# this-Demir/3D-Ray-Tracer-Vulkan

Hardware: AMD Instinct MI355X
Metric: Mrays/s at 1920×1080×4-bounce, 50k-tri scene; 1/2/4/8 GPU + %HBM roofline (higher is better)
Workload: dtype f32

## Files before the change

3d-ray-tracer-vulkan_amd/csrc/rt_trace.hip:

```cpp
#include <algorithm>
#include <cstdio>
#include <cstdlib>
#include <cstring>

#include "rt_internal.h"

namespace rtamd {

namespace {

constexpr float kTMin = 0.001f;
constexpr float kTMax = 10000.0f;
constexpr int   kMaxRejectTriples = 1 << 16;

struct V3 { float x, y, z; };

__device__ __forceinline__ V3 vadd(V3 a, V3 b) { return {a.x + b.x, a.y + b.y, a.z + b.z}; }
__device__ __forceinline__ V3 vsub(V3 a, V3 b) { return {a.x - b.x, a.y - b.y, a.z - b.z}; }
__device__ __forceinline__ V3 vmul(V3 a, V3 b) { return {a.x * b.x, a.y * b.y, a.z * b.z}; }
__device__ __forceinline__ V3 vscale(V3 a, float s) { return {a.x * s, a.y * s, a.z * s}; }
__device__ __forceinline__ float vdot(V3 a, V3 b) { return (a.x * b.x + a.y * b.y) + a.z * b.z; }
__device__ __forceinline__ V3 vcross(V3 a, V3 b) {
    return {a.y * b.z - a.z * b.y, a.z * b.x - a.x * b.z, a.x * b.y - a.y * b.x};
}
__device__ __forceinline__ V3 vnormalize(V3 a) {
    const float l = sqrtf(vdot(a, a));
    return {a.x / l, a.y / l, a.z / l};
}

__device__ __forceinline__ uint32_t pcg(uint32_t v) {
    const uint32_t s = v * 747796405u + 2891336453u;
    const uint32_t w = ((s >> ((s >> 28u) + 4u)) ^ s) * 277803737u;
    return (w >> 22u) ^ w;
}
__device__ __forceinline__ float rnd(uint32_t& seed) {
    seed = pcg(seed);
    return (float)seed / 4294967296.0f;
}

__device__ __forceinline__ V3 rnd_in_sphere(uint32_t& seed) {
    seed = pcg(pcg(pcg(seed)));
    for (int it = 0; it < kMaxRejectTriples; ++it) {
        const float a = rnd(seed);
        const float b = rnd(seed);
        const float c = rnd(seed);
        const V3 p = {a * 2.0f - 1.0f, b * 2.0f - 1.0f, c * 2.0f - 1.0f};
        if (vdot(p, p) < 1.0f) return p;
    }
    return {0.0f, 0.0f, 0.0f};
}

__device__ __forceinline__ uint8_t unorm8(float c) {
    return c > 0.0f ? (c < 1.0f ? (uint8_t)__builtin_rintf(c * 255.0f) : (uint8_t)255) : (uint8_t)0;
}

__device__ __forceinline__ int frame_row(const TraceArgs& a, int f, int ly) {
    if (a.band_list) return a.y0 + a.band_list[f * a.list_stride + ly / a.band_h] * a.band_h + ly % a.band_h;
    return a.y0 + ((ly / a.band_h) * a.band_stride + a.band_off) * a.band_h + ly % a.band_h;
}

__device__ __forceinline__ void primary_ray_seeded(const TraceArgs& a, int f, int x, int y, uint32_t& seed, V3& o,
                                                   V3& d);
__device__ __forceinline__ void primary_ray(const TraceArgs& a, int f, int x, int y, uint32_t& seed, V3& o, V3& d) {
    seed = (uint32_t)(y * a.width + x);
    primary_ray_seeded(a, f, x, y, seed, o, d);
}

__device__ __forceinline__ void primary_ray_seeded(const TraceArgs& a, int f, int x, int y, uint32_t& seed, V3& o,
                                                   V3& d) {
    const float u = ((float)x + rnd(seed)) / (float)a.width;
    const float v = ((float)(a.height - 1 - y) + rnd(seed)) / (float)a.height;
    const CamF& c = a.cams[f];
    const V3 cam_o = {c.ox, c.oy, c.oz};
    const V3 cam_l = {c.lx, c.ly, c.lz};
    const V3 cam_h = {c.hx, c.hy, c.hz};
    const V3 cam_v = {c.vx, c.vy, c.vz};
    o = cam_o;
    d = vnormalize(vsub(vadd(vadd(cam_l, vscale(cam_h, u)), vscale(cam_v, v)), cam_o));
}

typedef float f2 __attribute__((ext_vector_type(2)));

__device__ __forceinline__ void slab(float4 A, float4 B, V3 o, V3 inv, float& te, bool& ind) {
    const f2 oxy = {o.x, o.y}, ixy = {inv.x, inv.y};
    const f2 t0 = (f2{A.x, A.y} - oxy) * ixy;
    const f2 t1 = (f2{B.x, B.y} - oxy) * ixy;
    const float t0x = t0.x, t1x = t1.x, t0y = t0.y, t1y = t1.y;
    const float t0z = (A.z - o.z) * inv.z, t1z = (B.z - o.z) * inv.z;
    te = fmaxf(fmaxf(fminf(t0x, t1x), fminf(t0y, t1y)), fminf(t0z, t1z));
    const float tx = fminf(fminf(fmaxf(t0x, t1x), fmaxf(t0y, t1y)), fmaxf(t0z, t1z));
    ind = tx > te && tx > kTMin;
}

__device__ __forceinline__ bool tri_test(float4 P0, float4 P1, float4 P2, V3 o, V3 d, float& t) {
    const V3 v0 = {P0.x, P0.y, P0.z};
    const V3 e1 = {P1.x, P1.y, P1.z};
    const V3 e2 = {P2.x, P2.y, P2.z};
    const V3 pv = vcross(d, e2);
    const float det = vdot(e1, pv);
    if (det > -0.00001f && det < 0.00001f) return false;
    const float inv_det = 1.0f / det;
    const V3 s = vsub(o, v0);
    const float uu = inv_det * vdot(s, pv);
    if (uu < 0.0f || uu > 1.0f) return false;
    const V3 q = vcross(s, e1);
    const float vv = inv_det * vdot(d, q);
    if (vv < 0.0f || (uu + vv) > 1.0f) return false;
    t = inv_det * vdot(e2, q);
    return t > kTMin;
}

__device__ __forceinline__ void pin(float4& q) { asm volatile("" : "+v"(q.x), "+v"(q.y), "+v"(q.z), "+v"(q.w)); }

template <bool COUNT>
__device__ __forceinline__ int node_step(const float4* __restrict__ nodes, const float4* __restrict__ leafs,
                                         int i, bool& leaf, V3 o, V3 d, V3 inv, float& closest, int& hit,
                                         unsigned long long& c_node, unsigned long long& c_tri) {
    const float4 A = nodes[2 * i];
    const float4 B = nodes[2 * i + 1];
    float4 P0, P1, P2;
    if (leaf) {
        P0 = leafs[3 * i + 0];
        P1 = leafs[3 * i + 1];
        P2 = leafs[3 * i + 2];
        pin(P0);
        pin(P1);
        pin(P2);
    }
    float te;
    bool ind;
    slab(A, B, o, inv, te, ind);
    const bool hb = ind && te < closest;
    if (COUNT && hb && !leaf) c_node += 2;
    if (hb && leaf) {
        if (COUNT) ++c_tri;
        float t;
        if (tri_test(P0, P1, P2, o, d, t) && t < closest) {
            closest = t;
            hit = __float_as_int(P0.w);
        }
    }
    const uint32_t aw = __float_as_uint(A.w), bw = __float_as_uint(B.w);
    leaf = hb ? (bw & 1u) : (aw >> 31);
    return hb ? i + 1 : (int)(aw & 0x7FFFFFFFu);
}

__device__ __forceinline__ V3 hit_normal(const float4* __restrict__ norms, int hit, V3 d) {
    const float4 N = norms[kShadeStride * hit];
    V3 n = {N.x, N.y, N.z};
    if (vdot(d, n) > 0.0f) n = {-n.x, -n.y, -n.z};
    return n;
}

__device__ __forceinline__ void sphere_tests(const float4* __restrict__ sph, int n, V3 o, V3 d,
                                             float& closest, int& hit) {
    const float qa = vdot(d, d);
    for (int k = 0; k < n; ++k) {
        const float4 S = sph[2 * k];
        const V3 oc = {o.x - S.x, o.y - S.y, o.z - S.z};
        const float hb = vdot(oc, d);
        const float qc = vdot(oc, oc) - S.w * S.w;
        const float disc = hb * hb - qa * qc;
        if (!(disc >= 0.0f)) continue;
        const float sq = sqrtf(disc);
        float root = (-hb - sq) / qa;
        if (!(root > kTMin && root < closest)) {
            root = (-hb + sq) / qa;
            if (!(root > kTMin && root < closest)) continue;
        }
        closest = root;
        hit = -2 - k;
    }
}

__device__ __forceinline__ V3 sphere_normal(float4 S, V3 hp, V3 d) {
    V3 n = {(hp.x - S.x) / S.w, (hp.y - S.y) / S.w, (hp.z - S.z) / S.w};
    if (vdot(d, n) > 0.0f) n = {-n.x, -n.y, -n.z};
    return n;
}

__device__ __forceinline__ bool scatter(float4 M, V3 d, V3 n, uint32_t& seed, V3& nd) {
    if (M.w == 0.0f) {
        const V3 ru = vnormalize(rnd_in_sphere(seed));
        V3 sd = vadd(n, ru);
        if (sqrtf(vdot(sd, sd)) < 0.0001f) sd = n;
        nd = vnormalize(sd);
        return true;
    }
    if (M.w == 1.0f || M.w == 2.0f) {
        const float fuzz = (M.w == 2.0f) ? 0.3f : 0.0f;
        const V3 di = vnormalize(d);
        const float k = 2.0f * vdot(n, di);
        const V3 refl = vsub(di, vscale(n, k));
        const V3 p = rnd_in_sphere(seed);
        nd = vnormalize(vadd(refl, vscale(p, fuzz)));
        return vdot(nd, n) > 0.0f;
    }
    nd = d;
    return false;
}

__device__ __forceinline__ V3 sky_color(V3 d) {
    const V3 ud = vnormalize(d);
    const float t = 0.5f * (ud.y + 1.0f);
    const float omt = 1.0f - t;
    return {omt * 1.0f + t * 0.5f, omt * 1.0f + t * 0.7f, omt * 1.0f + t * 1.0f};
}

__device__ __forceinline__ void write_pixel(const TraceArgs& a, int lx, int ly, V3 fin) {
    const V3 g = {sqrtf(fin.x), sqrtf(fin.y), sqrtf(fin.z)};
    const size_t p = (size_t)ly * (size_t)a.tw + (size_t)lx;
    if (a.out_rgba) a.out_rgba[p] = make_uchar4(unorm8(g.x), unorm8(g.y), unorm8(g.z), 255);
    if (a.out_rad) {
        a.out_rad[3 * p + 0] = g.x;
        a.out_rad[3 * p + 1] = g.y;
        a.out_rad[3 * p + 2] = g.z;
    }
}

constexpr int kFeatExtBit = 16;

template <int FEAT>
__device__ __forceinline__ void finish_pixel(const TraceArgs& a, int lx, int ly, V3 fin) {
    if ((FEAT & kFeatExtBit) && a.out_lin) {
        float* lin = a.out_lin + 3 * ((size_t)ly * (size_t)a.tw + (size_t)lx);
        lin[0] = fin.x;
        lin[1] = fin.y;
        lin[2] = fin.z;
        return;
    }
    if ((FEAT & kFeatExtBit) && (a.ext & kExtAccumulate)) {
        float* acc = a.accum + 3 * ((size_t)ly * (size_t)a.tw + (size_t)lx);
        const float nf = (float)(a.frame_count + 1);
        const V3 sum = a.frame_count == 0 ? fin : V3{acc[0] + fin.x, acc[1] + fin.y, acc[2] + fin.z};
        acc[0] = sum.x;
        acc[1] = sum.y;
        acc[2] = sum.z;
        fin = {sum.x / nf, sum.y / nf, sum.z / nf};
    }
    write_pixel(a, lx, ly, fin);
}

__device__ __forceinline__ void flush_counters(Counters* c, unsigned long long s, unsigned long long n,
                                               unsigned long long t, unsigned long long m) {
// ... 346 lines not shown
        const uint64_t CI = __ballot(cand && !lf);
        if (room < 2 && ((CI >> k) & 1ull)) {
            pos = lane_i(node, k);
            pos_leaf = false;
            return false;
        }
        const bool sel = cand && (lf || lane == k || 2 * (lanes_below(CI) + 1) <= room - kFReserve);
        bool hL = false, hR = false;
        uint4 cL = e, cR = e;
        if (sel) {
            if (lf) {
                const float4 P0 = leafs[3 * node + 0];
                const float4 P1 = leafs[3 * node + 1];
                const float4 P2 = leafs[3 * node + 2];
                float t;
                const bool v = tri_test(P0, P1, P2, o, d, t);
                e.y = __float_as_uint(P0.w);
                e.w = v ? __float_as_uint(t) : 0x7F800000u;
            } else {
                const float4 Q0 = pairs[4 * node + 0];
                const float4 Q1 = pairs[4 * node + 1];
                const float4 Q2 = pairs[4 * node + 2];
                const float4 Q3 = pairs[4 * node + 3];
                float teL, teR;
                bool indL, indR;
                slab(Q0, Q1, o, inv, teL, indL);
                slab(make_float4(Q0.w, Q1.w, Q2.w, 0.f), Q2, o, inv, teR, indR);
                const uint32_t rw = __float_as_uint(Q3.x);
                hL = indL && teL < closest;
                hR = indR && teR < closest;
                cL = make_uint4((uint32_t)(node + 1) | (__float_as_uint(Q3.y) != 0u ? 0x80000000u : 0u), rw & kIdx,
                                __float_as_uint(teL), kUnres);
                cR = make_uint4(rw, e.y, __float_as_uint(teR), kUnres);
                e.w = 0u;
            }
        }
        const bool reg = in && lane >= k;
        const uint64_t RM = __ballot(reg), LM = __ballot(hL), RRM = __ballot(hR);
        const int P = lanes_below(RM) + lanes_below(LM) + lanes_below(RRM);
        const int ntop = top - (nl - k) + __popcll(RM) + __popcll(LM) + __popcll(RRM);
        if (reg) {
            F[ntop - 1 - P] = e;
            if (hL) F[ntop - 2 - P] = cL;
            if (hR) F[ntop - 2 - (hL ? 1 : 0) - P] = cR;
        }
        top = ntop;
    }
    pos = end;
    return true;
}


__device__ __forceinline__ void diag_stamp(unsigned long long* rec, int which) {
    unsigned long long t;
    asm volatile("s_memrealtime %0\n\ts_waitcnt lgkmcnt(0)" : "=s"(t) :: "memory");
    if ((threadIdx.x & 63) == 0) {
        rec[which] = t;
        if (which == 0) {
            unsigned hw, xcc;
            asm volatile("s_getreg_b32 %0, hwreg(HW_REG_HW_ID)" : "=s"(hw));
            asm volatile("s_getreg_b32 %0, hwreg(HW_REG_XCC_ID)" : "=s"(xcc));
            rec[2] = ((unsigned long long)xcc << 32) | hw;
            rec[3] = ((unsigned long long)(blockIdx.y * gridDim.x + blockIdx.x) << 8) | (threadIdx.x >> 6);
        }
    }
}

constexpr int kDiagWords = 8;
constexpr int kFeatCoopTail = 8;
constexpr int kFeatExt = kFeatExtBit;
constexpr int kFeatFrontier = 32;

constexpr int kFeatFused = 64;
constexpr int kFeatWin32 = 128;
constexpr int kFeatPad = 256;
constexpr int kFeatQ1 = 4096;
constexpr int kFeatQ2 = 8192;
constexpr int kFeatHalf = 2048;
constexpr int kFeatWide = 1024;
constexpr int kFeatAccel = 512;
constexpr int kFeatQuery = 16384;
constexpr int kFeatSolo = 32768;
constexpr unsigned kHeavyLaneMark = kLearnHeavyMark;

__device__ __forceinline__ void store_hit(float4* h, float t, int tri, V3 n, V3 p) {
    h[0] = make_float4(t, __int_as_float(tri), n.x, n.y);
    h[1] = make_float4(n.z, p.x, p.y, p.z);
}
__device__ __forceinline__ bool finite3(V3 a) {
    return fabsf(a.x) < __builtin_inff() && fabsf(a.y) < __builtin_inff() && fabsf(a.z) < __builtin_inff();
}

template <bool COUNT>
__device__ __forceinline__ void heavy_pixel(const TraceArgs& a, int f, int lx, int ly, int lyo, uint4* F) {
    const int lane = threadIdx.x & 63;
    const int end = a.scene.end;
    unsigned long long c_seg = 0, c_node = 0, c_tri = 0, c_mat = 0;
    if (lx < a.tw && ly < a.th && (a.list_stride == 0 || a.band_list[f * a.list_stride + ly / a.band_h] >= 0)) {
        uint32_t seed;
        V3 o, d;
        primary_ray(a, f, a.x0 + lx, frame_row(a, f, ly), seed, o, d);
        V3 att = {1.0f, 1.0f, 1.0f};
        V3 fin = {0.0f, 0.0f, 0.0f};
        int rounds = 0;
        for (int b = 0; b < a.max_bounces; ++b) {
            float closest = kTMax;
            int hit = -1;
            const V3 inv = {1.0f / d.x, 1.0f / d.y, 1.0f / d.z};
            if (COUNT) {
                ++c_seg;
                if (end > 0) ++c_node;
            }
            if (end > 0) {
                int p = 0;
                bool pl = false;
                if (!frontier_walk<COUNT>(a.scene.nodes, a.scene.leafs, a.scene.pairs, end, p, pl, o, d, inv, closest,
                                          hit, c_node, c_tri, F, rounds))
                    while (p < end) p = node_step<COUNT>(a.scene.nodes, a.scene.leafs, p, pl, o, d, inv, closest, hit,
                                                         c_node, c_tri);
            }
            if (hit < 0) {
                fin = vmul(att, sky_color(d));
                break;
            }
            if (COUNT) ++c_mat;
            const V3 hp = vadd(o, vscale(d, closest));
            const V3 nrm = hit_normal(a.scene.norms, hit, d);
            const float4 M = a.scene.mats[kShadeStride * hit];
            V3 nd;
            if (!scatter(M, d, nrm, seed, nd)) break;
            att = vmul(att, V3{M.x, M.y, M.z});
            o = hp;
            d = nd;
        }
        if (lane == 0) write_pixel(a, lx, lyo, fin);
    }
    if (COUNT) {
        if (lane != 0) c_seg = c_node = c_tri = c_mat = 0;
        flush_counters(a.counters, c_seg, c_node, c_tri, c_mat);
    }
}

typedef uint32_t u32x8 __attribute__((ext_vector_type(8)));
__device__ __forceinline__ u32x8 srec(const float4* __restrict__ walk, unsigned byte) {
    typedef const __attribute__((address_space(4))) char* cbytes;
    return *(const __attribute__((address_space(4))) u32x8*)((cbytes)walk + byte);
}
template <bool COUNT, bool DIAG, bool QRY>
__device__ __forceinline__ void solo_walk(const float4* __restrict__ walk, int L, unsigned sb, unsigned se, bool sl,
                                          bool any_hit, V3 o, V3 d, V3 inv, float& closest, int& hit, bool& incons,
                                          float& lim, unsigned long long& c_node, unsigned long long& c_tri,
                                          unsigned long long& d_iters) {
    const bool me = (int)(threadIdx.x & 63) == L;
    unsigned cn = 0, ct = 0, steps = 0;
    for (;;) {
        const u32x8 R = srec(walk, sb);
        u32x8 T;
        if (sl) T = srec(walk, sb + 32u);
        const uint32_t aw = R[3], bw = R[7];
        float te;
        bool ind;
        slab(make_float4(__uint_as_float(R[0]), __uint_as_float(R[1]), __uint_as_float(R[2]), 0.f),
             make_float4(__uint_as_float(R[4]), __uint_as_float(R[5]), __uint_as_float(R[6]), 0.f), o, inv, te, ind);
        const bool hb = ((__ballot(ind && accel_enter_lim(te, lim, aw)) >> L) & 1ull) != 0ull;
        const unsigned tb = sb + (sl ? 64u : 32u);
        sb = (hb || sl) ? tb : (aw << 5);
        const bool nl = (hb && !sl) ? (int)bw < 0 : (int)aw < 0;
        if (COUNT && hb && !sl) cn += 2;
        if (DIAG) ++steps;
        if (hb && sl) {
            if (COUNT) ++ct;
            float t;
            const bool tv = tri_test(make_float4(__uint_as_float(bw), __uint_as_float(T[0]), __uint_as_float(T[1]), 0.f),
                                     make_float4(__uint_as_float(T[2]), __uint_as_float(T[3]), __uint_as_float(T[4]), 0.f),
                                     make_float4(__uint_as_float(T[5]), __uint_as_float(T[6]), __uint_as_float(T[7]), 0.f),
                                     o, d, t) &&
                            accel_take(t, (int)(aw & kTri), closest, hit);
            if (((__ballot(tv) >> L) & 1ull) != 0ull && me) {
                closest = t;
                hit = (int)(aw & kTri);
                incons = t < te;
                lim = accel_lim(t);
            }
        }
        sl = nl;
        if (!(sb < se)) break;
        if (QRY && any_hit && ((__ballot(hit >= 0 && !incons) >> L) & 1ull) != 0ull) break;
    }
    if (me) {
        if (COUNT) {
            c_node += cn;
            c_tri += ct;
        }
        if (DIAG) d_iters += steps;
    }
}

constexpr int kWavesPerEu = 8;
constexpr int kWalkPrio = 2;
template <bool COUNT, bool DIAG = false, int FEAT = 0, int WALK = 2>
__global__ __launch_bounds__(256)
__attribute__((amdgpu_waves_per_eu((FEAT & kFeatFrontier) ? 1 : kWavesPerEu)))
void trace_simple(TraceArgs a) {
    constexpr bool ACC = (FEAT & kFeatAccel) != 0;
    constexpr bool HALF = ACC && (FEAT & kFeatHalf) != 0;
    constexpr bool WIDE = ACC && (FEAT & kFeatWide) != 0;
    constexpr bool PAD = !ACC && ((FEAT & kFeatPad) || (FEAT & (kFeatExt | kFeatFrontier)) || !(FEAT & kFeatCoopTail));
    constexpr bool Q1 = (FEAT & kFeatQ1) != 0, Q2 = (FEAT & kFeatQ2) != 0;
    constexpr bool QRY = (FEAT & kFeatQuery) != 0;
    constexpr bool SOLO = (FEAT & kFeatSolo) != 0;
    static_assert(!SOLO || (ACC && !HALF && !WIDE && WALK == 2 && !(FEAT & (kFeatCoopTail | kFeatExt))),
                  "kFeatSolo goes with the format-0 accel walk alone");
    const int lane = threadIdx.x & 63;
    const int wave = threadIdx.x >> 6;
    extern __shared__ uint4 fr[];
    unsigned q_first = 0u, q_valid = 0u;
    if (Q2) {
        const unsigned q = blockIdx.x % (unsigned)a.q_queues;
        unsigned* const h = a.q_hdr + kQHdrWords * (size_t)q;
        const unsigned cnt = __hip_atomic_load(h + kQCount, __ATOMIC_RELAXED, __HIP_MEMORY_SCOPE_AGENT);
        const unsigned lim = ~__hip_atomic_load(h + kQLimit, __ATOMIC_RELAXED, __HIP_MEMORY_SCOPE_AGENT);
        asm volatile("s_waitcnt vmcnt(0)" ::: "memory");
        if (lane == 0) {
            const unsigned t = __hip_atomic_fetch_add(h + kQTicket, 1u, __ATOMIC_RELAXED, __HIP_MEMORY_SCOPE_AGENT);
            if (t + 1u == (unsigned)a.q_packs) {
                __hip_atomic_store(h + kQCount, 0u, __ATOMIC_RELAXED, __HIP_MEMORY_SCOPE_AGENT);
                __hip_atomic_store(h + kQLimit, 0u, __ATOMIC_RELAXED, __HIP_MEMORY_SCOPE_AGENT);
                __hip_atomic_store(h + kQTicket, 0u, __ATOMIC_RELAXED, __HIP_MEMORY_SCOPE_AGENT);
            }
        }
        q_valid = min(min(cnt, lim), (unsigned)a.q_cap);
        q_first = (blockIdx.x / (unsigned)a.q_queues) * 64u;
        if (q_first >= q_valid) return;
        q_first += q * (unsigned)a.q_cap;
        q_valid += q * (unsigned)a.q_cap;
    }
    const int s = a.wave_tile;
    const int tw_w = 8 << s, th_w = 8 >> s;
    int bx = blockIdx.x, by = blockIdx.y, sub = -1;
    if (QRY) {
        by = bx / a.tiles_x;
        bx -= by * a.tiles_x;
    }
    unsigned long long skip_lanes = 0;
    const int k_wave = (blockIdx.y * gridDim.x + blockIdx.x) * a.block_waves + wave;
    int rec_id = k_wave, tile_id = k_wave, hq = -1;
    if (a.tile_order) {
        const int k = blockIdx.x;
        int t;
        if ((FEAT & kFeatFused) && k < a.n_heavy_px) {
            hq = a.heavy_px[k];
            t = hq >> 6;
            sub = hq & 63;
        } else if (k < 64 * a.split_n) {
            t = a.tile_order[k >> 6];
            sub = k & 63;
        } else {
            t = a.tile_order[k - 63 * a.split_n - ((FEAT & kFeatFused) ? a.n_heavy_px : 0)];
            if ((FEAT & kFeatFused) && a.tile_mask) skip_lanes = a.tile_mask[t];
            if (FEAT & kFeatFused) {
                rec_id = a.n_heavy_px + t;
                tile_id = t;
            } else if (DIAG && a.diag_lane && a.split_n == 0) {
                rec_id = t;
                tile_id = t;
            }
        }
        bx = t % a.tiles_x;
        by = t / a.tiles_x;
    }
    unsigned long long* drec = nullptr;
    if (DIAG) {
        drec = a.diag + kDiagWords * (size_t)rec_id;
        diag_stamp(drec, 0);
    }
    if ((FEAT & kFeatFused) && sub >= 0) {
        const int hf = by / a.tiles_y;
        const int hy = (by - hf * a.tiles_y) * th_w + (sub >> (3 + s));
        heavy_pixel<COUNT>(a, hf, bx * tw_w + (sub & (tw_w - 1)), hy, (a.row_off ? a.row_off[hf] : hf * a.th) + hy, fr);
        if (DIAG) {
            diag_stamp(drec, 1);
            if (lane == 0) {
                drec[4] = 0;
                drec[5] = 0;
                drec[6] = 0;
                drec[7] = 0;
                if (a.diag_lane && hq >= 0) a.diag_lane[hq] = kHeavyLaneMark;
            }
        }
        return;
    }
    const int tl = sub >= 0 ? sub : lane;
    const int col = bx * a.block_waves + wave;
    const int fr_i = by / a.tiles_y;
    by -= fr_i * a.tiles_y;
    int lx = col * tw_w + (tl & (tw_w - 1));
    const int ly = by * th_w + (tl >> (3 + s));
    int lyo = (a.row_off ? a.row_off[fr_i] : fr_i * a.th) + ly;
    const bool pixel = !Q2 && lx < a.tw && ly < a.th && (sub < 0 || lane == 0) && !((skip_lanes >> lane) & 1ull) &&
                       (a.list_stride == 0 || a.band_list[fr_i * a.list_stride + ly / a.band_h] >= 0);
    const int coop_lanes = sub >= 0 ? 64 : a.coop_lanes;
    const float4* __restrict__ nodes = a.scene.nodes;
    const float4* __restrict__ leafs = a.scene.leafs;
    const float4* __restrict__ pairs = a.scene.pairs;
    const int end = a.scene.end;
    const int wend = WALK == 2 ? a.scene.end2 : end;
    unsigned long long c_seg = 0, c_node = 0, c_tri = 0, c_mat = 0;
    unsigned long long d_iters = 0, d_windows = 0, d_coop_t = 0;
    unsigned long long d_lane_windows = 0;

    uint32_t seed = 0;
    V3 o = {0.f, 0.f, 0.f}, d = {0.f, 0.f, 1.f};
    V3 att = {1.0f, 1.0f, 1.0f};
    bool alive = pixel;
    int b0 = 0;
    float tmax = kTMax;
    bool refq = false;
    if (Q2) {
        const unsigned i = q_first + (unsigned)lane;
        alive = i < q_valid;
        b0 = a.split_bounce;
        if (alive) {
            const float4* r = a.q_slots + 3 * (size_t)i;
            const float4 r0 = r[0], r1 = r[1], r2 = r[2];
            o = {r0.x, r0.y, r0.z};
            d = {r0.w, r1.x, r1.y};
            att = {r1.z, r1.w, r2.x};
            seed = __float_as_uint(r2.y);
            const unsigned pq = __float_as_uint(r2.z);
            alive = pq < a.q_pixels;
            lyo = (int)(pq / (unsigned)a.tw);
            lx = (int)(pq - (unsigned)lyo * (unsigned)a.tw);
        }
    }
    if (QRY && a.ray_in) {
        if (pixel) {
            const float4 r0 = a.ray_in[2 * (size_t)lx], r1 = a.ray_in[2 * (size_t)lx + 1];
            o = {r0.x, r0.y, r0.z};
            d = {r1.x, r1.y, r1.z};
            if (r0.w < kTMax) tmax = r0.w;
            if (!finite3(o) || !finite3(d) || (d.x == 0.0f && d.y == 0.0f && d.z == 0.0f)) {
                store_hit(a.hit_out + 2 * (size_t)lx, 0.0f, -2, V3{0.f, 0.f, 0.f}, V3{0.f, 0.f, 0.f});
                alive = false;
            }
            refq = ACC && fabsf(vdot(d, d) - 1.0f) > kRelaxAbs;
        }
    } else if (pixel) {
        const int x = a.x0 + lx, y = frame_row(a, fr_i, ly);
        if ((FEAT & kFeatExt) && (a.ext & (kExtAccumulate | kExtNewSample))) {
            seed = (uint32_t)(y * a.width + x) +
                   (uint32_t)(a.frame_count + fr_i * a.sample_step) * (uint32_t)(a.width * a.height);
            primary_ray_seeded(a, fr_i, x, y, seed, o, d);
        } else {
            primary_ray(a, fr_i, x, y, seed, o, d);
        }
    }

    for (int b = b0; b < (QRY ? 1 : a.max_bounces); ++b) {
        if (__ballot(alive) == 0) break;
        if (Q1 && b == a.split_bounce) {
            const uint64_t m = __ballot(alive);
            const unsigned n = (unsigned)__popcll(m);
            const unsigned q = (unsigned)k_wave % (unsigned)a.q_queues;
            unsigned* const h = a.q_hdr + kQHdrWords * (size_t)q;
            int base = 0;
            if (lane == 0)
                base = (int)__hip_atomic_fetch_add(h + kQCount, n, __ATOMIC_RELAXED, __HIP_MEMORY_SCOPE_AGENT);
            base = lane_i(base, 0);
            if ((unsigned long long)(unsigned)base + n <= (unsigned long long)(unsigned)a.q_cap) {
                if (alive) {
                    float4* r = a.q_slots + 3 * ((size_t)q * (size_t)a.q_cap + (unsigned)base + (size_t)lanes_below(m));
                    r[0] = make_float4(o.x, o.y, o.z, d.x);
                    r[1] = make_float4(d.y, d.z, att.x, att.y);
                    r[2] = make_float4(att.z, __uint_as_float(seed), __int_as_float(lyo * a.tw + lx), 0.0f);
                }
                alive = false;
                break;
            }
            if (lane == 0) {
                __hip_atomic_fetch_max(h + kQLimit, ~(unsigned)base, __ATOMIC_RELAXED, __HIP_MEMORY_SCOPE_AGENT);
                __hip_atomic_fetch_add(a.q_overflow, 1u, __ATOMIC_RELAXED, __HIP_MEMORY_SCOPE_AGENT);
            }
        }
        float closest = QRY ? tmax : kTMax;
        int hit = -1;
        const V3 inv = {1.0f / d.x, 1.0f / d.y, 1.0f / d.z};
        int n = 0;
        int lend = wend;
        bool incons = false;
        int oct = 0;
        if (ACC && a.scene.n_layouts == 8) {
            oct = (int)((__float_as_uint(d.x) >> 31) | ((__float_as_uint(d.y) >> 31) << 1) |
                        ((__float_as_uint(d.z) >> 31) << 2)) & a.scene.oct_mask;
            n = oct * a.scene.layout_slots;
            lend = n + a.scene.layout_slots;
        }
        bool nleaf = a.scene.root_leaf != 0;
        const bool own = alive && !(QRY && refq);
        bool walking = own && end > 0;
        if (ACC && !HALF && !WIDE && a.scene.root_enter) {
            n += 1;
            nleaf = ((a.scene.root_first_leaf >> oct) & 1) != 0;
            if (COUNT && own) c_node += 2;
        }
        uint32_t wcur = a.scene.root_leaf ? kWLeaf : 0u;
        int wsp = 0;
        bool wovf = false;
        if (COUNT && alive) {
            ++c_seg;
            if (end > 0 && own) ++c_node;
        }
        {
            float4 A, B, Q0, Q1;
            const float4* __restrict__ wr = a.scene.walk;
            const __amdgpu_buffer_rsrc_t wrs = __builtin_amdgcn_make_buffer_rsrc(
                const_cast<float4*>(wr), 0,
                WIDE ? (int)((unsigned)(a.scene.end2 + 1) * 64u)
                     : HALF ? (int)((unsigned)(a.scene.end2 + 4) * 16u) : (int)((unsigned)(a.scene.end2 + 2) * 32u),
                0x00020000);
            const bool walk0 = walking;
            if (SOLO && __popcll(__ballot(walking)) <= a.solo_lanes) walking = false;
            if (WIDE) {
            } else if (HALF && walking) {
                A = hbuf(wrs, n);
                if (nleaf) {
                    B = hbuf(wrs, n + 1);
                    Q0 = hbuf(wrs, n + 2);
                    Q1 = hbuf(wrs, n + 3);
                }
            } else if (WALK == 2 && walking) {
                A = wr[2 * n];
                B = wr[2 * n + 1];
                if (nleaf) {
                    Q0 = wr[2 * n + 2];
                    Q1 = wr[2 * n + 3];
                }
            }
            float lim = accel_lim(closest);
            __builtin_amdgcn_s_setprio(kWalkPrio);
            constexpr bool BYTES = ACC && !HALF && !WIDE && !PAD && WALK == 2;
            unsigned nb = (unsigned)n << 5;
            const unsigned lend_b = (unsigned)lend << 5;
            while (walking) {
                if (DIAG) ++d_iters;
                if (WIDE) {
                    walking = wide_step<COUNT>(wrs, fr + (size_t)wave * (kWideStackK * 64 * 6 / 16), o, d, inv, closest,
                                               hit, incons, wcur, wsp, wovf, c_node, c_tri);
                    continue;
                }
                if (WALK == 0) {
                    n = node_step<COUNT>(nodes, leafs, n, nleaf, o, d, inv, closest, hit, c_node, c_tri);
                } else if (HALF) {
                    const uint32_t aw = __float_as_uint(A.w);
                    const uint32_t h0 = __float_as_uint(A.x), h1 = __float_as_uint(A.y), h2 = __float_as_uint(A.z);
                    const float4 lo = nleaf ? A : make_float4(half_lo(h0), half_hi(h0), half_lo(h1), 0.f);
                    const float4 hi = nleaf ? B : make_float4(half_hi(h1), half_lo(h2), half_hi(h2), 0.f);
                    float te;
                    bool ind;
                    slab(lo, hi, o, inv, te, ind);
                    const float rf = nleaf ? ((aw & kThinLeaf) ? __builtin_inff() : kRelax) : a.scene.relax_half;
                    const bool hb = ind && accel_enter_r(te, closest, rf);
                    const int nxt = nleaf ? n + 4 : (hb ? n + 1 : (int)(aw & 0x3FFFFFFFu));
                    const bool nl = ((nleaf || !hb) ? (aw >> 31) : (aw >> 30)) & 1u;
                    const float v0x = B.w;
                    if (COUNT && hb && !nleaf) c_node += 2;
                    A = hbuf(wrs, nxt);
                    if (hb && nleaf) {
                        if (COUNT) ++c_tri;
                        float t;
                        if (tri_test(make_float4(v0x, Q0.x, Q0.y, 0.f), make_float4(Q0.z, Q0.w, Q1.x, 0.f),
                                     make_float4(Q1.y, Q1.z, Q1.w, 0.f), o, d, t) &&
                            accel_take(t, (int)(aw & kTri), closest, hit)) {
                            closest = t;
                            hit = (int)(aw & kTri);
                            incons = t < te;
                        }
                    }
                    if (nl && nxt < lend) {
                        B = hbuf(wrs, nxt + 1);
                        Q0 = hbuf(wrs, nxt + 2);
                        Q1 = hbuf(wrs, nxt + 3);
                    }
                    n = nxt;
                    nleaf = nl;
                } else {
                    float te;
                    bool ind;
                    slab(A, B, o, inv, te, ind);
                    const uint32_t aw = __float_as_uint(A.w), bw = __float_as_uint(B.w);
                    const bool hb = ind && (ACC ? accel_enter_lim(te, lim, aw) : te < closest);
                    int nxt;
                    if (PAD) {
                        const int n_leaf = n + 2 + (int)((aw >> 29) & 1u);
                        const int n_hit = n + 1 + (int)((bw >> 2) & 1u);
                        const int m_hit = -(int)hb, m_leaf = -(int)nleaf;
                        const int n_int = (n_hit & m_hit) | ((int)(aw & kIdx) & ~m_hit);
                        nxt = (n_leaf & m_leaf) | (n_int & ~m_leaf);
                    } else if (BYTES) {
                        const unsigned tb = nb + (nleaf ? 64u : 32u);
                        nb = (hb || nleaf) ? tb : (aw << 5);
                        nxt = 0;
                    } else {
                        const int t = n + 1 + (int)nleaf;
                        nxt = (hb || nleaf) ? t : (int)(aw & kIdx);
                    }
                    const bool nl = ACC ? ((hb && !nleaf) ? (int)bw < 0 : (int)aw < 0)
                                        : ((((hb && !nleaf) ? bw : (aw >> 31)) & 1u) != 0u);
                    const float v0x = B.w;
                    if (COUNT && hb && !nleaf) c_node += 2;
                    if (BYTES) {
                        A = wbuf_b(wrs, nb, 0);
                        B = wbuf_b(wrs, nb, 16);
                    } else {
                        A = wbuf(wrs, nxt, 0);
                        B = wbuf(wrs, nxt, 16);
                    }
                    if (hb && nleaf) {
                        if (COUNT) ++c_tri;
                        float t;
                        if (tri_test(make_float4(v0x, Q0.x, Q0.y, 0.f), make_float4(Q0.z, Q0.w, Q1.x, 0.f),
                                     make_float4(Q1.y, Q1.z, Q1.w, 0.f), o, d, t) &&
                            (ACC ? accel_take(t, (int)(aw & kTri), closest, hit) : t < closest)) {
                            closest = t;
                            hit = (int)(aw & kTri);
                            if (ACC) {
                                incons = t < te;
                                lim = accel_lim(t);
                            }
                        }
                    }
                    const bool inb = BYTES ? nb < lend_b : nxt < (ACC ? lend : wend);
                    if (nl && inb) {
                        if (BYTES) {
                            Q0 = wbuf_b(wrs, nb, 32);
                            Q1 = wbuf_b(wrs, nb, 48);
                        } else {
                            Q0 = wbuf(wrs, nxt, 32);
                            Q1 = wbuf(wrs, nxt, 48);
                        }
                    }
                    if (!BYTES) n = nxt;
                    nleaf = nl;
                    walking = inb;
                    if (QRY && a.any_hit && hit >= 0 && !incons) walking = false;
                }
                if (WALK == 0 || HALF) walking = n < (ACC ? lend : wend);
                if ((FEAT & kFeatCoopTail) && __popcll(__ballot(walking)) <= coop_lanes) break;
                if (SOLO) walking = walking && __popcll(__ballot(walking)) > a.solo_lanes;
            }
            if (SOLO) {
                uint64_t rem = __ballot(walk0 && nb < lend_b && !(QRY && a.any_hit && hit >= 0 && !incons));
                while (rem != 0) {
                    const int L = __ffsll((long long)rem) - 1;
                    rem &= rem - 1;
                    solo_walk<COUNT, DIAG, QRY>(wr, L, (unsigned)lane_i((int)nb, L), (unsigned)lane_i((int)lend_b, L),
                                                lane_i((int)nleaf, L) != 0, QRY && a.any_hit, o, d, inv, closest, hit,
                                                incons, lim, c_node, c_tri, d_iters);
                }
                walking = false;
            }
            if (BYTES) n = (int)(nb >> 5);
            __builtin_amdgcn_s_setprio(0);
        }
        if (FEAT & kFeatCoopTail) {
            uint64_t rem = __ballot(walking);
            unsigned long long tc0 = 0;
            if (DIAG && rem != 0) tc0 = wall_clock64();
            while (rem != 0) {
                const int L = __ffsll((long long)rem) - 1;
                rem &= rem - 1;
                const V3 bo = {lane_f(o.x, L), lane_f(o.y, L), lane_f(o.z, L)};
                const V3 bd = {lane_f(d.x, L), lane_f(d.y, L), lane_f(d.z, L)};
                const V3 bi = {lane_f(inv.x, L), lane_f(inv.y, L), lane_f(inv.z, L)};
                float bc = lane_f(closest, L);
                int bh = lane_i(hit, L);
                bool bx = ACC && lane_i((int)incons, L) != 0;
                unsigned long long cn = 0, ct = 0;
                const int start = n;
                int nw = 0;
                if ((FEAT & kFeatFrontier) && a.coop_walk) {
                    int p = WALK == 2 ? a.scene.slot_node[lane_i(start, L)] : lane_i(start, L);
                    bool pl = false;
                    if (!frontier_walk<COUNT>(nodes, leafs, pairs, end, p, pl, bo, bd, bi, bc, bh, cn, ct,
                                              fr + wave * kFCap, nw))
                        while (p < end) p = node_step<COUNT>(nodes, leafs, p, pl, bo, bd, bi, bc, bh, cn, ct);
                } else {
                    const int ws = WALK == 2 ? lane_i(start, L) : a.scene.node_slot[lane_i(start, L)];
                    nw = coop_walk<COUNT, (FEAT & kFeatWin32) ? 32 : 64, PAD, ACC>(
                        a.scene.walk, ACC ? lane_i(lend, L) : a.scene.end2, ws, bo, bd, bi, bc, bh, cn, ct, bx);
                }
                if (DIAG) {
                    d_windows += nw;
                    if (lane == L) d_lane_windows += nw;
                }
                if (lane == L) {
                    closest = bc;
                    hit = bh;
                    if (ACC) incons = bx;
                    if (COUNT) {
                        c_node += cn;
                        c_tri += ct;
                    }
                }
            }
            if (DIAG && tc0) d_coop_t += wall_clock64() - tc0;
        }
        if (ACC) {
            uint64_t redo = __ballot(alive && ((hit >= 0 && incons) || (WIDE && wovf) || (QRY && refq)));
            while (redo != 0) {
                const int L = __ffsll((long long)redo) - 1;
                redo &= redo - 1;
                const V3 bo = {lane_f(o.x, L), lane_f(o.y, L), lane_f(o.z, L)};
                const V3 bd = {lane_f(d.x, L), lane_f(d.y, L), lane_f(d.z, L)};
                const V3 bi = {lane_f(inv.x, L), lane_f(inv.y, L), lane_f(inv.z, L)};
                float bc = QRY ? lane_f(tmax, L) : kTMax;
                int bh = -1;
                bool bx = false;
                unsigned long long cn = 1, ct = 0;
                coop_walk<COUNT, (FEAT & kFeatWin32) ? 32 : 64, true, false>(a.scene.walk_ref, a.scene.end2_ref, 0,
                                                                             bo, bd, bi, bc, bh, cn, ct, bx);
                if (lane == L) {
                    closest = bc;
                    hit = bh;
                    if (COUNT) {
                        c_node += cn;
                        c_tri += ct;
                    }
                }
            }
        }
        if ((FEAT & kFeatExt) && alive && a.scene.n_spheres > 0)
            sphere_tests(a.scene.spheres, a.scene.n_spheres, o, d, closest, hit);
        if (QRY && alive) {
            float4* h = a.hit_out + 2 * ((size_t)lyo * (size_t)a.tw + (size_t)lx);
            if (hit >= 0)
                store_hit(h, closest, hit, hit_normal(a.scene.norms, hit, d), vadd(o, vscale(d, closest)));
            else
                store_hit(h, tmax, -1, V3{0.f, 0.f, 0.f}, V3{0.f, 0.f, 0.f});
            alive = false;
        }
        if (!QRY && alive) {
            V3 fin = {0.0f, 0.0f, 0.0f};
            if ((FEAT & kFeatExt) ? hit != -1 : hit >= 0) {
                if (COUNT) ++c_mat;
                const V3 hp = vadd(o, vscale(d, closest));
                V3 nrm;
                float4 M;
                if ((FEAT & kFeatExt) && hit < -1) {
                    nrm = sphere_normal(a.scene.spheres[2 * (-2 - hit)], hp, d);
                    M = a.scene.spheres[2 * (-2 - hit) + 1];
                } else {
                    nrm = hit_normal(a.scene.norms, hit, d);
                    M = a.scene.mats[kShadeStride * hit];
                }
                V3 nd;
                if ((FEAT & kFeatExt) && (a.ext & kExtEmissive) && M.w == 3.0f) {
                    fin = vmul(att, V3{M.x, M.y, M.z});
                    alive = false;
                } else if (!scatter(M, d, nrm, seed, nd)) {
                    alive = false;
                } else {
                    att = vmul(att, V3{M.x, M.y, M.z});
                    o = hp;
                    d = nd;
                    if (b == a.max_bounces - 1) alive = false;
                }
            } else {
                if (!((FEAT & kFeatExt) && (a.ext & kExtSkyToggle) && a.sky_enabled == 0))
                    fin = vmul(att, sky_color(d));
                alive = false;
            }
            if (!alive) finish_pixel<FEAT>(a, lx, lyo, fin);
        }
    }
    if (!QRY && alive) finish_pixel<FEAT>(a, lx, lyo, V3{0.0f, 0.0f, 0.0f});
    if (COUNT) flush_counters(a.counters, c_seg, c_node, c_tri, c_mat);
    if (DIAG) {
        diag_stamp(drec, 1);
        if (a.diag_lane && !((skip_lanes >> lane) & 1ull))
            a.diag_lane[(size_t)tile_id * 64 + lane] = (unsigned)(d_iters + 2 * d_lane_windows);
        unsigned long long d_sum = d_iters;
#pragma unroll
        for (int off = 32; off > 0; off >>= 1) {
            d_sum += __shfl_xor(d_sum, off);
            const unsigned long long o2 = __shfl_xor(d_iters, off);
            d_iters = o2 > d_iters ? o2 : d_iters;
        }
        if (lane == 0) {
            drec[4] = d_iters;
            drec[5] = d_windows;
            drec[6] = d_coop_t;
            drec[7] = d_sum;
        }
    }
}

}

#define RT_FUSED(G)                                                                                           \
    if (a.diag) hipLaunchKernelGGL((trace_simple<false, true, FF, 2>), G, block, shm, stream, ao);             \
    else if (a.counters) hipLaunchKernelGGL((trace_simple<true, false, FF, 2>), G, block, shm, stream, ao);     \
// ... 201 lines not shown
```

Before: 34730.

## Split BYTES BVH walk into dedicated loop and streamline solo walk ballots

```diff
diff --git a/3d-ray-tracer-vulkan_amd/csrc/rt_trace.hip b/3d-ray-tracer-vulkan_amd/csrc/rt_trace.hip
--- a/3d-ray-tracer-vulkan_amd/csrc/rt_trace.hip
+++ b/3d-ray-tracer-vulkan_amd/csrc/rt_trace.hip
@@ -81,15 +81,20 @@
 
 typedef float f2 __attribute__((ext_vector_type(2)));
 
+__device__ __forceinline__ void slab_t(float4 A, float4 B, V3 o, V3 inv, float& te, float& tx);
 __device__ __forceinline__ void slab(float4 A, float4 B, V3 o, V3 inv, float& te, bool& ind) {
+    float tx;
+    slab_t(A, B, o, inv, te, tx);
+    ind = tx > te && tx > kTMin;
+}
+__device__ __forceinline__ void slab_t(float4 A, float4 B, V3 o, V3 inv, float& te, float& tx) {
     const f2 oxy = {o.x, o.y}, ixy = {inv.x, inv.y};
     const f2 t0 = (f2{A.x, A.y} - oxy) * ixy;
     const f2 t1 = (f2{B.x, B.y} - oxy) * ixy;
     const float t0x = t0.x, t1x = t1.x, t0y = t0.y, t1y = t1.y;
     const float t0z = (A.z - o.z) * inv.z, t1z = (B.z - o.z) * inv.z;
     te = fmaxf(fmaxf(fminf(t0x, t1x), fminf(t0y, t1y)), fminf(t0z, t1z));
-    const float tx = fminf(fminf(fmaxf(t0x, t1x), fmaxf(t0y, t1y)), fmaxf(t0z, t1z));
-    ind = tx > te && tx > kTMin;
+    tx = fminf(fminf(fmaxf(t0x, t1x), fmaxf(t0y, t1y)), fmaxf(t0z, t1z));
 }
 
 __device__ __forceinline__ bool tri_test(float4 P0, float4 P1, float4 P2, V3 o, V3 d, float& t) {
@@ -742,23 +747,28 @@
                                           float& lim, unsigned long long& c_node, unsigned long long& c_tri,
                                           unsigned long long& d_iters) {
     const bool me = (int)(threadIdx.x & 63) == L;
+    const uint64_t lbit = 1ull << L;
     unsigned cn = 0, ct = 0, steps = 0;
+    unsigned lf = sl ? 1u : 0u;
     for (;;) {
         const u32x8 R = srec(walk, sb);
         u32x8 T;
-        if (sl) T = srec(walk, sb + 32u);
+        if (lf) T = srec(walk, sb + 32u);
         const uint32_t aw = R[3], bw = R[7];
-        float te;
-        bool ind;
-        slab(make_float4(__uint_as_float(R[0]), __uint_as_float(R[1]), __uint_as_float(R[2]), 0.f),
-             make_float4(__uint_as_float(R[4]), __uint_as_float(R[5]), __uint_as_float(R[6]), 0.f), o, inv, te, ind);
-        const bool hb = ((__ballot(ind && accel_enter_lim(te, lim, aw)) >> L) & 1ull) != 0ull;
-        const unsigned tb = sb + (sl ? 64u : 32u);
-        sb = (hb || sl) ? tb : (aw << 5);
-        const bool nl = (hb && !sl) ? (int)bw < 0 : (int)aw < 0;
-        if (COUNT && hb && !sl) cn += 2;
+        float te, tx;
+        slab_t(make_float4(__uint_as_float(R[0]), __uint_as_float(R[1]), __uint_as_float(R[2]), 0.f),
+               make_float4(__uint_as_float(R[4]), __uint_as_float(R[5]), __uint_as_float(R[6]), 0.f), o, inv, te, tx);
+        const uint64_t forced = (aw & kForce) != 0u ? ~0ull : 0ull;
+        const uint64_t m = __builtin_amdgcn_ballot_w64(tx > te) & __builtin_amdgcn_ballot_w64(tx > kTMin) &
+                           (__builtin_amdgcn_ballot_w64(te <= lim) | forced);
+        const unsigned hb = (unsigned)(m >> L) & 1u;
+        const unsigned tb = sb + 32u + (lf << 5);
+        sb = (hb | lf) ? tb : (aw << 5);
+        const unsigned first = hb & ~lf;
+        const uint32_t nw = first ? bw : aw;
+        if (COUNT && first) cn += 2;
         if (DIAG) ++steps;
-        if (hb && sl) {
+        if (hb & lf) {
             if (COUNT) ++ct;
             float t;
             const bool tv = tri_test(make_float4(__uint_as_float(bw), __uint_as_float(T[0]), __uint_as_float(T[1]), 0.f),
@@ -766,16 +776,16 @@
                                      make_float4(__uint_as_float(T[5]), __uint_as_float(T[6]), __uint_as_float(T[7]), 0.f),
                                      o, d, t) &&
                             accel_take(t, (int)(aw & kTri), closest, hit);
-            if (((__ballot(tv) >> L) & 1ull) != 0ull && me) {
+            if ((__builtin_amdgcn_ballot_w64(tv) & lbit) != 0ull && me) {
                 closest = t;
                 hit = (int)(aw & kTri);
                 incons = t < te;
                 lim = accel_lim(t);
             }
         }
-        sl = nl;
+        lf = nw >> 31;
         if (!(sb < se)) break;
-        if (QRY && any_hit && ((__ballot(hit >= 0 && !incons) >> L) & 1ull) != 0ull) break;
+        if (QRY && any_hit && (__builtin_amdgcn_ballot_w64(hit >= 0 && !incons) & lbit) != 0ull) break;
     }
     if (me) {
         if (COUNT) {
@@ -1030,8 +1040,56 @@
             __builtin_amdgcn_s_setprio(kWalkPrio);
             constexpr bool BYTES = ACC && !HALF && !WIDE && !PAD && WALK == 2;
             unsigned nb = (unsigned)n << 5;
-            const unsigned lend_b = (unsigned)lend << 5;
-            while (walking) {
+            const unsigned lend_b = walk0 ? (unsigned)lend << 5 : 0u;
+            if (BYTES) {
+                uint32_t lw = nleaf ? 0x80000000u : 0u;
+                const int keep = SOLO ? a.solo_lanes : ((FEAT & kFeatCoopTail) ? coop_lanes : 0);
+                bool w = walking;
+                if (__ballot(w) != 0ull) {
+                    do {
+                        if (w) {
+                            if (DIAG) ++d_iters;
+                            float te;
+                            bool ind;
+                            slab(A, B, o, inv, te, ind);
+                            const uint32_t aw = __float_as_uint(A.w), bw = __float_as_uint(B.w);
+                            const bool lf = (int)lw < 0;
+                            const bool hb = ind && accel_enter_lim(te, lim, aw);
+                            const unsigned tb = nb + (lf ? 64u : 32u);
+                            nb = (hb || lf) ? tb : (aw << 5);
+                            const bool hl = hb && lf;
+                            lw = (hb != hl) ? bw : aw;
+                            float v0x;
+                            asm volatile("v_mov_b32 %0, %2" : "=v"(v0x), "+v"(lw) : "v"(B.w));
+                            if (COUNT && hb && !lf) c_node += 2;
+                            A = wbuf_b(wrs, nb, 0);
+                            B = wbuf_b(wrs, nb, 16);
+                            if (hl) {
+                                if (COUNT) ++c_tri;
+                                float t;
+                                const int tri = (int)(lw & kTri);
+                                if (tri_test(make_float4(v0x, Q0.x, Q0.y, 0.f), make_float4(Q0.z, Q0.w, Q1.x, 0.f),
+                                             make_float4(Q1.y, Q1.z, Q1.w, 0.f), o, d, t) &&
+                                    accel_take(t, tri, closest, hit)) {
+                                    closest = t;
+                                    hit = tri;
+                                    incons = t < te;
+                                    lim = accel_lim(t);
+                                }
+                            }
+                            if ((int)lw < 0 && nb < lend_b) {
+                                Q0 = wbuf_b(wrs, nb, 32);
+                                Q1 = wbuf_b(wrs, nb, 48);
+                            }
+                        }
+                        w = nb < lend_b;
+                        if (QRY) w = w && !(a.any_hit && hit >= 0 && !incons);
+                    } while (__popcll(__ballot(w)) > keep);
+                }
+                walking = w;
+                nleaf = (int)lw < 0;
+            }
+            while (!BYTES && walking) {
                 if (DIAG) ++d_iters;
                 if (WIDE) {
                     walking = wide_step<COUNT>(wrs, fr + (size_t)wave * (kWideStackK * 64 * 6 / 16), o, d, inv, closest,
@@ -1086,10 +1144,6 @@
                         const int m_hit = -(int)hb, m_leaf = -(int)nleaf;
                         const int n_int = (n_hit & m_hit) | ((int)(aw & kIdx) & ~m_hit);
                         nxt = (n_leaf & m_leaf) | (n_int & ~m_leaf);
-                    } else if (BYTES) {
-                        const unsigned tb = nb + (nleaf ? 64u : 32u);
-                        nb = (hb || nleaf) ? tb : (aw << 5);
-                        nxt = 0;
                     } else {
                         const int t = n + 1 + (int)nleaf;
                         nxt = (hb || nleaf) ? t : (int)(aw & kIdx);
@@ -1098,13 +1152,8 @@
                                         : ((((hb && !nleaf) ? bw : (aw >> 31)) & 1u) != 0u);
                     const float v0x = B.w;
                     if (COUNT && hb && !nleaf) c_node += 2;
-                    if (BYTES) {
-                        A = wbuf_b(wrs, nb, 0);
-                        B = wbuf_b(wrs, nb, 16);
-                    } else {
-                        A = wbuf(wrs, nxt, 0);
-                        B = wbuf(wrs, nxt, 16);
-                    }
+                    A = wbuf(wrs, nxt, 0);
+                    B = wbuf(wrs, nxt, 16);
                     if (hb && nleaf) {
                         if (COUNT) ++c_tri;
                         float t;
@@ -1119,24 +1168,18 @@
                             }
                         }
                     }
-                    const bool inb = BYTES ? nb < lend_b : nxt < (ACC ? lend : wend);
+                    const bool inb = nxt < (ACC ? lend : wend);
                     if (nl && inb) {
-                        if (BYTES) {
-                            Q0 = wbuf_b(wrs, nb, 32);
-                            Q1 = wbuf_b(wrs, nb, 48);
-                        } else {
-                            Q0 = wbuf(wrs, nxt, 32);
-                            Q1 = wbuf(wrs, nxt, 48);
-                        }
+                        Q0 = wbuf(wrs, nxt, 32);
+                        Q1 = wbuf(wrs, nxt, 48);
                     }
-                    if (!BYTES) n = nxt;
+                    n = nxt;
                     nleaf = nl;
                     walking = inb;
                     if (QRY && a.any_hit && hit >= 0 && !incons) walking = false;
                 }
                 if (WALK == 0 || HALF) walking = n < (ACC ? lend : wend);
                 if ((FEAT & kFeatCoopTail) && __popcll(__ballot(walking)) <= coop_lanes) break;
-                if (SOLO) walking = walking && __popcll(__ballot(walking)) > a.solo_lanes;
             }
             if (SOLO) {
                 uint64_t rem = __ballot(walk0 && nb < lend_b && !(QRY && a.any_hit && hit >= 0 && !incons));
```

New measurement: 36480 (median of 6 runs). 1.05x the previous value.
